# serhii-rieznik/metal-renderer

Hardware: AMD Instinct MI355X
Metric: Mpaths/s at 1920×1080, 4 bounces; achieved HBM GB/s vs peak; 1/2/4/8-GPU scaling (higher is better)
Workload: dtype f32

## Files before the change

### include/mrt.h

```cpp
#ifndef MRT_H_
#define MRT_H_

#include <stddef.h>
#include <stdint.h>

#ifdef __cplusplus
extern "C" {
#endif

#define MRT_ABI_VERSION 9

typedef enum mrt_status {
  MRT_OK = 0,
  MRT_ERR_INVALID = -1,
  MRT_ERR_IO = -2,
  MRT_ERR_HIP = -3,
  MRT_ERR_NOMEM = -4,
  MRT_ERR_STATE = -5,
  MRT_ERR_COMM = -6
} mrt_status;

#define MRT_FLAG_PRECISE 1u
#define MRT_FLAG_PROFILE 2u
#define MRT_FLAG_STATIC_NOISE 4u
// ... 188 lines not shown
int mrt_renderer_destroy(mrt_renderer* r);

const char* mrt_last_error(void);
int mrt_abi_version(void);
int mrt_noise_table(uint64_t seed, int64_t frame, float* out16384);
int mrt_shard_mask(uint32_t width, uint32_t height, uint32_t shard_rank, uint32_t shard_count, uint8_t* mask,
                   uint64_t* owned);
#define MRT_DISPLAY_TONEMAP 1u
#define MRT_DISPLAY_SRGB 2u
#define MRT_DISPLAY_DENOISED 4u
#define MRT_DISPLAY_RESOLVED 8u
#define MRT_DISPLAY_COMPARE(mode) ((uint32_t)(mode) << 8)
int mrt_display(const float* image, const float* reference, float* out, uint32_t width, uint32_t height,
                uint32_t flags, float compare_scale, void* stream);

int mrt_image_load_exr(const char* path, float* rgba, size_t capacity_floats, uint32_t* width, uint32_t* height);
int mrt_renderer_load_reference(mrt_renderer* r, const char* path);
int mrt_renderer_display(mrt_renderer* r, uint32_t flags, float compare_scale, float* rgba, size_t count);
#define MRT_DISPLAY_SLOTS 3u
int mrt_renderer_display_enqueue(mrt_renderer* r, uint32_t flags, float compare_scale, uint32_t slot);
int mrt_renderer_display_map(mrt_renderer* r, uint32_t slot, const float** rgba, size_t* count);

int mrt_tiles_packed_floats(uint32_t width, uint32_t height, uint32_t shard_rank, uint32_t shard_count,
                            uint64_t* floats);
int mrt_tiles_pack(const float* image, uint32_t width, uint32_t height, uint32_t shard_rank,
                   uint32_t shard_count, float* packed, void* stream);
int mrt_tiles_unpack(const float* packed, uint32_t width, uint32_t height, uint32_t shard_rank,
                     uint32_t shard_count, float* image, void* stream);
#define MRT_COMM_ID_BYTES 128
#define MRT_EXCHANGE_GATHER 1u
#define MRT_EXCHANGE_REDUCE 2u
#define MRT_EXCHANGE_OVERLAP 0x100u
typedef struct mrt_comm mrt_comm;
int mrt_comm_unique_id(void* id, size_t bytes);
int mrt_comm_create(const void* id, uint32_t nranks, uint32_t rank, int device, mrt_comm** out);
int mrt_comm_destroy(mrt_comm* comm);
int mrt_renderer_exchange(mrt_renderer* r, mrt_comm* comm, uint32_t mode);
int mrt_renderer_exchange_flush(mrt_renderer* r);
int mrt_comm_set_timeout(mrt_comm* comm, uint32_t timeout_ms);
int mrt_comm_check(mrt_comm* comm);
int mrt_debug_comm_fail(mrt_comm* comm, uint32_t mode);
int mrt_renderer_tiles_read(mrt_renderer* r, float* host_packed, size_t floats);
int mrt_renderer_tiles_write(mrt_renderer* r, uint32_t shard_rank, const float* host_packed, size_t floats);

int mrt_synchronize(void* stream);
int mrt_event_record(void* stream, void** event);
int mrt_event_synchronize(void* event);
int mrt_event_destroy(void* event);
int mrt_debug_stamps(uint64_t* out8, int reset);
int mrt_debug_wave_times(uint64_t* out, size_t n);
int mrt_debug_lanes(uint64_t* out, size_t n, int reset);
int mrt_debug_sweep_list(const mrt_scene* scene, float* records, uint32_t capacity, uint32_t* count,
                         uint32_t* enabled);
int mrt_debug_sweep_cap(const mrt_scene* scene, uint32_t* cap);
int mrt_debug_bvh_nodes(const mrt_scene* scene, float* nodes, uint32_t capacity, uint32_t* count);
int mrt_debug_exchange_unpack(mrt_renderer* r, uint32_t nranks, const float* gathered, size_t floats);
int mrt_debug_box_margin(const mrt_scene* scene, const void* rays, uint32_t stride, uint32_t count,
                         const void* intersections, float* out);
int mrt_debug_magic_div(uint32_t d, const uint32_t* n, uint32_t count, uint32_t* q);
int mrt_debug_denoise_path(uint32_t path);
int mrt_debug_denoise_step(const float* image, const float* guide_n, const float* guide_p, float* out, float* scratch,
                           uint32_t width, uint32_t height, const mrt_denoise_params* params, uint32_t step_log2,
                           uint32_t path, void* stream);
int mrt_device_count(void);

#ifdef __cplusplus
}
#endif
#endif
```

### metal-renderer_amd/csrc/kernels.hip

```cpp
#include <hip/hip_runtime.h>
#include <math.h>

#include <algorithm>
#include <cstdlib>
#include <vector>

#include "diag_env.h"
#include "kernels.h"

#ifndef MRT_PRECISE
#error "compile with -DMRT_PRECISE=0 or 1"
#endif
#ifndef MRT_TU
#define MRT_TU 0
#endif
#ifndef MRT_LANESTATS
#define MRT_LANESTATS 0
#endif
#define MRT_EMIT_STREAM (MRT_TU == 0 || (MRT_TU == 2 && !MRT_LANESTATS) || (MRT_TU == 1 && MRT_LANESTATS))
#define MRT_EMIT_MAIN (MRT_TU != 2)
#if MRT_PRECISE
#define MRT_NS precise
#else
#define MRT_NS fast
// ... 290 lines not shown
  return (int32_t)v;
}

template <int MODE>
__device__ __forceinline__ LdsCtx stage_lds(const DeviceScene& sc, uint32_t scratch_u32, uint32_t* spill = nullptr) {
  LdsCtx cx;
  const uint32_t nf4 = node_float4s(sc.width);
  const uint32_t n_nodes = (MODE == kAllLds) ? scene_nodes(sc) : (MODE == kTopLds ? sc.lds_nodes : 0u);
  const uint32_t TR = (MODE == kAllLds) ? scene_tri_records(sc) : 0u;
  const uint32_t T = (MODE == kAllLds) ? sc.num_triangles : 0u;
  const uint32_t M = (MODE == kAllLds) ? sc.num_materials : 0u;
  const uint32_t NL = (MODE == kAllLds) ? sc.num_lights + 1 : 0u;
  const uint32_t SW = (MODE == kAllLds) ? sc.sweep_leaves : 0u;
  cx.n_lds_nodes = n_nodes;
  const uint32_t node_f4 = node_stride_f4(MODE, nf4);
  const bool copies = node_f4 != nf4;
  cx.tri_base = node_f4 * n_nodes;
  cx.prim_base = cx.tri_base + 3 * TR;
  cx.mat_base = cx.prim_base + 6 * T;
  cx.light_base = cx.mat_base + 2 * M;
  cx.sweep_base = cx.light_base + 7 * NL;
  const uint32_t f4 = cx.sweep_base + 2 * SW;
  cx.scratch_base = 4 * f4;
  cx.stack_base = cx.scratch_base + ((scratch_u32 + 3) & ~3u);
  cx.spill_lane = sc.max_stack;
  cx.spill = spill ? spill + (size_t)blockIdx.x * kBlock * cx.spill_lane : nullptr;
  if (MODE != kGlobal) {
    const float4* src[6] = {reinterpret_cast<const float4*>(sc.nodes), reinterpret_cast<const float4*>(sc.tris),
                            reinterpret_cast<const float4*>(sc.prims), reinterpret_cast<const float4*>(sc.materials),
                            reinterpret_cast<const float4*>(sc.lights), reinterpret_cast<const float4*>(sc.sweep)};
    const uint32_t base[6] = {0u, cx.tri_base, cx.prim_base, cx.mat_base, cx.light_base, cx.sweep_base};
    const uint32_t len[6] = {nf4 * n_nodes, 3 * TR, 6 * T, 2 * M, 7 * NL, 2 * SW};
    for (int r = copies ? 1 : 0; r < 6; ++r)
      for (uint32_t i = threadIdx.x; i < len[r]; i += kBlock) g_lds[base[r] + i] = src[r][i];
    if (copies) {
      for (uint32_t i = threadIdx.x; i < node_f4 * n_nodes; i += kBlock) {
        const uint32_t node = i / node_f4, rem = i % node_f4;
        const uint32_t quad = rem / kQuadCopyF4, row = rem % kQuadCopyF4;
        const uint32_t axis = row >> 1;
        const uint32_t flip = axis < 2 ? (quad >> axis) & 1u : 0u;
        const uint32_t src_row = row < 6 ? 2 * axis + ((row & 1u) ^ flip) : 6u;
        g_lds[i] = src[0][8 * node + src_row];
      }
    }
    __syncthreads();
  }
  return cx;
}

#ifndef MRT_LANESTATS
#define MRT_LANESTATS 0
#endif
#if MRT_LANESTATS
constexpr int kLaneStats = 46;
__shared__ unsigned long long s_lanes[kBlock / 64][kLaneStats];
__device__ unsigned long long g_lanes[kLaneStats];
__device__ __forceinline__ void ls_add(int k, uint32_t v) {
  const uint64_t m = __ballot(1);
  if ((threadIdx.x & 63u) == (uint32_t)(__ffsll((unsigned long long)m) - 1)) s_lanes[threadIdx.x >> 6][k] += v;
}
__device__ __forceinline__ uint32_t ls_lanes() { return (uint32_t)__popcll(__ballot(1)); }
#define LS_ADD(k, v) ls_add((k), (v))
#define LS_INIT() do { if ((threadIdx.x & 63u) < (uint32_t)kLaneStats) s_lanes[threadIdx.x >> 6][threadIdx.x & 63u] = 0; } while (0)
#define LS_FLUSH() do { const uint32_t l_ = threadIdx.x & 63u; \
    if (l_ < (uint32_t)kLaneStats && s_lanes[threadIdx.x >> 6][l_]) atomicAdd(&g_lanes[l_], s_lanes[threadIdx.x >> 6][l_]); } while (0)
__device__ __forceinline__ uint64_t ls_clock() {
  uint64_t t;
  asm volatile("s_memtime %0\n\ts_waitcnt lgkmcnt(0)" : "=s"(t)::"memory");
  return t;
}
#define LS_T0() const uint64_t ls_t0_ = ls_clock()
#define LS_T1(k) do { LS_ADD((k), (uint32_t)(ls_clock() - ls_t0_)); LS_ADD((k) + 1, 1); } while (0)
#define LS_WAIT_VM(k) do { LS_T0(); asm volatile("s_waitcnt vmcnt(0)" ::: "memory"); LS_T1(k); } while (0)
#else
#define LS_ADD(k, v) do {} while (0)
#define LS_INIT() do {} while (0)
#define LS_FLUSH() do {} while (0)
#define LS_T0() do {} while (0)
#define LS_T1(k) do {} while (0)
#define LS_WAIT_VM(k) do {} while (0)
#endif

constexpr int32_t kDone = 0x7FFFFFFF;
#ifndef MRT_PATH_SLACK
#define MRT_PATH_SLACK 16
#endif
#ifndef MRT_LEAF_SLACK
#define MRT_LEAF_SLACK 12
#endif

template <int STACK>
__device__ __forceinline__ int32_t stack_pop(const LdsCtx& cx, int& sp) {
  if (STACK < 0 && !__any(sp > (STACK < 0 ? -STACK : STACK))) {
    const int32_t n = sp > 0 ? (int32_t)lds_u32()[cx.stack_base + threadIdx.x + (sp - 1) * kBlock] : kDone;
    sp = max(sp - 1, 0);
    return n;
  }
  const int32_t n = sp > 0 ? stack_get<STACK>(cx, sp - 1) : kDone;
  sp = max(sp - 1, 0);
  return n;
}

[[maybe_unused]] constexpr float kCullScale = 1.0f + 0x1p-11f;
template <int STACK, int MODE, bool ANY>
__device__ __forceinline__ int32_t interior_step(const DeviceScene& sc, const LdsCtx& cx, int32_t node, V3 o,
                                                 const RayBox& rb, float tmin, float tmax, int& sp) {
  {
// ... 101 lines not shown
  h.prim = 0xFFFFFFFFu;
  h.found = false;
  for (uint32_t j = 0; j < cnt; j += 2) {
    const uint32_t j1 = min(j + 1, cnt - 1);
#if MRT_LANESTATS
    const uint64_t t0_ = ls_clock();
    const uint32_t e0_ = list[j], e1_ = list[j1];
    asm volatile("s_waitcnt lgkmcnt(0)" ::"s"(e0_), "s"(e1_) : "memory");
    LS_ADD(38, (uint32_t)(ls_clock() - t0_));
#endif
    tri_pair<MODE>(sc, cx, o, d, 0.0f, list[j], list[j1], j1 != j, h, false, 0u, nullptr);
  }
}

template <int STACK, int MODE, bool ANY>
__device__ __forceinline__ bool traverse(const DeviceScene& sc, const LdsCtx& cx, V3 o, V3 d, float tmin, Hit& h,
                                         uint32_t target, int32_t root) {
  const RayBox rb = make_raybox(o, d);
  int32_t node = root, leaf = 0;
  int sp = 0;
  constexpr int kLs = ANY ? 6 : 0;
  (void)kLs;
  LS_ADD(kLs + 0, ls_lanes());
  LS_ADD(kLs + 1, 1);
  if (node < 0) { leaf = node; node = kDone; }
  while (node != kDone || leaf != 0) {
    while (node != kDone && node >= 0) {
      LS_ADD(kLs + 2, 1);
      LS_ADD(kLs + 3, ls_lanes());
      node = interior_step<STACK, MODE, ANY>(sc, cx, node, o, rb, tmin, h.t, sp);
      if (node < 0 && leaf == 0) {
        leaf = node;
        node = stack_pop<STACK>(cx, sp);
      }
      if (__ballot(leaf == 0) == 0ull) break;
    }
    while (leaf < 0) {
      LS_ADD(kLs + 4, 1);
      LS_ADD(kLs + 5, ls_lanes());
      const uint32_t lr = ~(uint32_t)leaf;
      const uint32_t first = lr >> kLeafCountBits, cnt = (lr & (kMaxLeafSize - 1)) + 1;
      if (leaf_tests<MODE>(sc, cx, o, d, tmin, first, cnt, h, ANY, target, nullptr)) return true;
      leaf = 0;
      if (node < 0) {
        leaf = node;
        node = stack_pop<STACK>(cx, sp);
      }
    }
  }
  return false;
}


__device__ __forceinline__ bool sweep_box(float4 lo, float4 hi, V3 o, const RayBox& rb, float tmin, float& tnear) {
#if MRT_PRECISE
  const float ox = o.x, oy = o.y, oz = o.z, oix = 0.0f, oiy = 0.0f, oiz = 0.0f;
#else
  const float ox = 0.0f, oy = 0.0f, oz = 0.0f, oix = rb.oinv.x, oiy = rb.oinv.y, oiz = rb.oinv.z;
  (void)o;
#endif
  const float x0 = slab(lo.x, ox, rb.inv.x, oix), x1 = slab(hi.x, ox, rb.inv.x, oix);
  const float y0 = slab(lo.y, oy, rb.inv.y, oiy), y1 = slab(hi.y, oy, rb.inv.y, oiy);
  const float z0 = slab(lo.z, oz, rb.inv.z, oiz), z1 = slab(hi.z, oz, rb.inv.z, oiz);
  tnear = fmaxf(fmaxf(fminf(x0, x1), fminf(y0, y1)), fmaxf(fminf(z0, z1), tmin));
  const float tfar = fminf(fminf(fmaxf(x0, x1), fmaxf(y0, y1)), fmaxf(z0, z1));
  return tnear <= tfar;
}

typedef float SweepRec __attribute__((ext_vector_type(8)));
typedef const __attribute__((address_space(4))) SweepRec* SweepList;

template <int MODE>
__device__ __forceinline__ void sweep_leaf(const DeviceScene& sc, const LdsCtx& cx, V3 o, V3 d, float tmin,
                                           uint32_t ref, Hit& h) {
  LS_ADD(4, 1);
  LS_ADD(5, ls_lanes());
  const uint32_t lr = ~ref;
  leaf_tests<MODE>(sc, cx, o, d, tmin, lr >> kLeafCountBits, (lr & (kMaxLeafSize - 1)) + 1, h, false, 0u, nullptr);
}

template <int MODE, bool CAP = false>
__device__ __forceinline__ uint32_t sweep_nearest(const DeviceScene& sc, const LdsCtx& cx, V3 o, V3 d, float tmin,
                                                  Hit& h, uint32_t cap = 0xFFFFFFFFu, uint32_t resume = 0u) {
  const RayBox rb = make_raybox(o, d);
  LS_ADD(0, ls_lanes());
  LS_ADD(1, 1);
  constexpr uint32_t kNone = 0xFFFFFFFFu;
  uint32_t k1 = kNone, k2 = kNone, rest = 0u;
  const uint32_t n = sc.sweep_leaves;
  const SweepList list = (SweepList)(uintptr_t)sc.sweep;
  for (uint32_t i = 0; i < n; ++i) {
    LS_T0();
    const SweepRec rec = list[i];
#if MRT_LANESTATS
    asm volatile("" ::"s"(rec[0]), "s"(rec[7]));
    LS_T1(42);
#endif
    float te;
    const bool hit = sweep_box(make_float4(rec[0], rec[1], rec[2], rec[3]), make_float4(rec[4], rec[5], rec[6], rec[7]),
                               o, rb, tmin, te);
    const uint32_t key = hit ? ((fbits(te) & ~31u) | (i & 31u)) : kNone;
    const uint32_t mid = max(k1, key);
    k1 = min(k1, key);
    k2 = min(k2, mid);
    rest |= (hit ? 1u : 0u) << (i & 31u);
  }
  rest &= ~((1u << (k1 & 31u)) | (1u << (k2 & 31u)));
  auto pop = [&](uint32_t& ref) {
    const uint32_t id = (uint32_t)__ffs((int)rest) - 1u;
    rest &= rest - 1u;
    const float4 blo = g_lds[cx.sweep_base + 2u * id], bhi = g_lds[cx.sweep_base + 2u * id + 1u];
    float te;
    ref = fbits(blo.w);
    return sweep_box(blo, bhi, o, rb, tmin, te) && te <= h.t * kCullScale;
  };
  if (!CAP) {
    if (k1 != kNone) sweep_leaf<MODE>(sc, cx, o, d, tmin, fbits(g_lds[cx.sweep_base + 2u * (k1 & 31u)].w), h);
    if (k2 != kNone && bitsf(k2 & ~31u) <= h.t * kCullScale)
      sweep_leaf<MODE>(sc, cx, o, d, tmin, fbits(g_lds[cx.sweep_base + 2u * (k2 & 31u)].w), h);
  } else {
    if (resume) rest = resume;
#pragma unroll
    for (int round = 0; round < 2; ++round) {
      const uint32_t k = round == 0 ? k1 : k2;
      bool test = k != kNone && (round == 0 || bitsf(k & ~31u) <= h.t * kCullScale);
      uint32_t ref = 0u;
      if (resume) {
        test = false;
        if (rest) test = pop(ref);
      } else if (test) {
        ref = fbits(g_lds[cx.sweep_base + 2u * (k & 31u)].w);
      }
      if (test) sweep_leaf<MODE>(sc, cx, o, d, tmin, ref, h);
    }
  }
  for (uint32_t c = 0; rest && (!CAP || c < cap); ++c) {
    LS_ADD(30, 1);
    LS_ADD(31, ls_lanes());
    uint32_t ref;
    if (pop(ref)) sweep_leaf<MODE>(sc, cx, o, d, tmin, ref, h);
  }
  return CAP ? rest : 0u;
}

template <int STACK, int MODE>
__device__ __forceinline__ Hit trace_nearest(const DeviceScene& sc, const LdsCtx& cx, V3 o, V3 d, float tmin,
                                             float tmax) {
  Hit h;
  h.t = tmax;
  h.u = h.v = 0.0f;
  h.prim = 0xFFFFFFFFu;
  h.found = false;
  if (MODE == kAllLds && sc.sweep_leaves) {
    sweep_nearest<MODE>(sc, cx, o, d, tmin, h);
    return h;
  }
  traverse<STACK, MODE, false>(sc, cx, o, d, tmin, h, 0u, sc.root);
  return h;
}

__device__ __forceinline__ int32_t shadow_root(const DeviceScene& sc, V3 o, bool graze) {
  const int32_t main_root = __builtin_amdgcn_readfirstlane(sc.root);
  if (sc.occ_planes == 0) return main_root;
  const int32_t occ_root = __builtin_amdgcn_readfirstlane(sc.occ_root);
  bool inside = !graze;
  for (uint32_t k = 0; k < sc.occ_planes; ++k) {
    const float* p = sc.occ_plane[k];
    inside &= fmaf(p[0], o.x, fmaf(p[1], o.y, fmaf(p[2], o.z, -p[3]))) <= -sc.occ_margin;
  }
  return inside ? occ_root : main_root;
}
__device__ __forceinline__ int32_t shadow_root_select(const DeviceScene& sc, V3 o, bool graze) {
  if (sc.occ_planes == 0 || graze) return sc.root;
  bool inside = true;
  for (uint32_t k = 0; k < sc.occ_planes; ++k) {
    const float* p = sc.occ_plane[k];
    inside &= fmaf(p[0], o.x, fmaf(p[1], o.y, fmaf(p[2], o.z, -p[3]))) <= -sc.occ_margin;
  }
  return inside ? sc.occ_root : sc.root;
}

template <int MODE>
__device__ __forceinline__ bool lights_occlude(const DeviceScene& sc, const LdsCtx& cx, V3 o, V3 d, uint32_t target,
                                               uint32_t tl, float tT) {
  bool occ = false;
  for (uint32_t j = 0; j + 1 < sc.num_lights; ++j) {
// ... 1872 lines not shown
```

### metal-renderer_amd/csrc/renderer.cpp

```cpp
#include <hip/hip_runtime.h>
#include <rccl/rccl.h>

#include <algorithm>
#include <atomic>
#include <chrono>
#include <cmath>
#include <cstdio>
#include <cstdlib>
#include <cstring>
#include <memory>
#include <mutex>
#include <string>
#include <thread>
#include <vector>

#include "../../include/mrt.h"
#include "bvh.h"
#include "bvh_gpu.h"
#include "denoise.h"
#include "temporal.h"
#include "image.h"
#include "kernels.h"
#include "noise.h"
#include "noise_schedule.h"
#include "occluders.h"
#include "primary.h"
#include "scene.h"
#include "diag_env.h"

namespace {

thread_local std::string g_last_error;

int fail(int code, const std::string& msg) {
  g_last_error = msg;
  return code;
}

#define HIP_TRY(expr)                                                                             \
  do {                                                                                            \
    hipError_t e_ = (expr);                                                                       \
    if (e_ != hipSuccess)                                                                         \
      return fail(MRT_ERR_HIP, std::string(#expr) + ": " + hipGetErrorString(e_));                \
  } while (0)

inline float bitsf(uint32_t u) { float f; std::memcpy(&f, &u, 4); return f; }
inline uint32_t fbits(float f) { uint32_t u; std::memcpy(&u, &f, 4); return u; }

struct DevBuf {
  void* p = nullptr;
  size_t bytes = 0;
  ~DevBuf() { if (p) (void)hipFree(p); }
  hipError_t alloc(size_t n) {
    if (p) { (void)hipFree(p); p = nullptr; }
    bytes = n;
    return n ? hipMalloc(&p, n) : hipSuccess;
  }
  template <class T> T* as() const { return reinterpret_cast<T*>(p); }
};

hipError_t alloc_isect_spill(DevBuf& b, uint32_t max_stack) {
  if (max_stack <= (uint32_t)mrt::kMaxStack) return b.alloc(0);
  return b.alloc((size_t)max_stack * mrt::kIntersectSpillGrid * 256 * 4);
}

#define NCCL_TRY(expr)                                                                            \
  do {                                                                                            \
    ncclResult_t e_ = (expr);                                                                     \
    if (e_ != ncclSuccess)                                                                        \
      return fail(MRT_ERR_HIP, std::string(#expr) + ": " + ncclGetErrorString(e_));               \
  } while (0)

hipError_t upload(DevBuf& b, const void* src, size_t n) {
  hipError_t e = b.alloc(std::max<size_t>(n, 16));
  if (e != hipSuccess) return e;
  return n ? hipMemcpy(b.p, src, n, hipMemcpyHostToDevice) : hipSuccess;
}

}

struct mrt_accel {
  mrt_accel_desc desc{};
  DevBuf nodes, tris;
  DevBuf isect_spill;
  mrt::DeviceScene dev{};
  mrt_accel_info info{};
};

struct mrt_scene {
  int device = 0;
  DevBuf isect_spill;
  mrt::HostScene host;
  mrt::BvhResult bvh;
  std::vector<float> occ_nodes, occ_tris;
  std::vector<uint32_t> occ_keep;
  int32_t occ_root = 0;
  uint32_t occ_node_base = 0, occ_max_stack = 0;
  DevBuf nodes, tris, prims, materials, lights;
  std::vector<float> sweep_list;
  bool sweep_on = false;
  uint32_t sweep_cap = mrt::kSweepCap;
  DevBuf sweep;
  mrt::DeviceScene dev{};
  mrt_scene_info info{};
};

struct DrawRecord {
  DevBuf counters;
  hipEvent_t start = nullptr, stop = nullptr;
  hipEvent_t cleared = nullptr;
  hipEvent_t copied = nullptr;
  void* host = nullptr;
  void* host_dev = nullptr;
  size_t host_bytes = 0;
  std::vector<hipEvent_t> kernel_events;
  uint32_t frames = 0;
  uint32_t launches = 0;
  size_t span_off = 0;
  size_t counter_bytes = 0;
  size_t events = 0;
  bool pending = false;
  bool clean = false;
};
constexpr int kDrawRing = 3;

struct FrameSlot {
  hipStream_t stream = nullptr;
  bool own_stream = false;
  DevBuf queue[2][mrt::kQueuePlanes];
  DevBuf segments;
  DevBuf radiance;
  DevBuf spill;
  hipEvent_t acc_done = nullptr;
  hipEvent_t kernel_done = nullptr;
  bool acc_recorded = false;
};

struct CameraGen {
  DevBuf dev;
  void* host = nullptr;
  size_t host_bytes = 0;
  hipEvent_t ready = nullptr;
  hipEvent_t retired = nullptr;
  bool busy = false;
  bool async = false;
  uint32_t waited_streams = 0;
  bool moved = false;
  bool has_lists = false;
  uint32_t primary_bx = 0;
  ~CameraGen() {
    if (ready) (void)hipEventDestroy(ready);
    if (retired) (void)hipEventDestroy(retired);
// ... 781 lines not shown
      occ_root = mrt::kEmptyChild;
    } else {
      if (ob.num_nodes) up_nodes.insert(up_nodes.end(), ob.nodes.begin(), ob.nodes.begin() + 32 * (size_t)ob.num_nodes);
      up_tris.insert(up_tris.end(), ob.tris.begin(), ob.tris.end());
      s->occ_nodes.assign(ob.nodes.begin(), ob.nodes.begin() + 32 * (size_t)ob.num_nodes);
      s->occ_tris = ob.tris;
      s->occ_keep = occ.keep;
      s->occ_root = occ_root;
      s->occ_node_base = node_base;
      s->occ_max_stack = ob.max_stack;
    }
  }
  mrt::ConvexSet conv;
  bool conv_on = occ_on && occ_lights && occ_root != mrt::kEmptyChild;
  if (const char* v = mrt::diag_env("MRT_CONVEX")) conv_on = conv_on && std::atoi(v) != 0;
  if (conv_on)
    conv_on = mrt::find_convex_occluders(h.vertices.data()->v, sizeof(mrt::RefVertex), (uint32_t)h.vertices.size(),
                                         h.indices.data(), T, occ.keep, occ, conv);
  if (conv_on)
    for (uint32_t t = 0; t < T; ++t) {
      const uint32_t code = conv.prim_face[t];
      prims[(size_t)t * 24 + 11] = bitsf(code);
      if (code)
        for (int c = 0; c < 3; ++c) prims[(size_t)t * 24 + 15 + 4 * c] = conv.face_normal[(code - 1) / 8][3 * ((code - 1) % 8) + c];
    }
  mrt_scene_info& in = s->info;
  if (conv_on) {
    in.convex_solids = conv.count;
    in.convex_delta = conv.delta;
    for (uint32_t c = 0; c < conv.count; ++c) {
      for (int i = 0; i < 16; ++i) in.convex_obb[c][i] = conv.obb[c][i];
      for (int k = 0; k < 8; ++k) in.convex_face_tris[c][k] = conv.face_tris[c][k];
    }
  }
  if (occ_on) {
    in.occluder_planes = (uint32_t)occ.planes.size();
    in.occluder_culled = occ.culled;
    in.occluder_nodes = ob.num_nodes;
    in.occluder_margin = occ.margin;
    in.occluder_max_stack = ob.max_stack;
    in.occluder_cos_min = occ.cos_min;
    for (size_t k = 0; k < occ.planes.size() && k < 8; ++k)
      for (int c = 0; c < 4; ++c) in.occluder_plane[k][c] = occ.planes[k][c];
  }
  if (s->bvh.root >= 0 && s->bvh.num_leaves <= mrt::kSweepLeaves) {
    for (uint32_t k = 0; k < s->bvh.num_nodes; ++k) {
      const float* nd = &s->bvh.nodes[32 * (size_t)k];
      for (int c = 0; c < 4; ++c)
        if ((int32_t)fbits(nd[24 + c]) < 0)
          s->sweep_list.insert(s->sweep_list.end(), {nd[c], nd[8 + c], nd[16 + c], nd[24 + c],
                                                     nd[4 + c], nd[12 + c], nd[20 + c], 0.0f});
    }
  }
  const uint32_t sweep_leaves = (uint32_t)(s->sweep_list.size() / 8);
  const uint32_t up_occ_nodes = occ_on ? (uint32_t)(up_nodes.size() / 32) - s->bvh.num_nodes : 0u;
  if (sweep_leaves >= 1 && sweep_leaves <= mrt::kSweepLeaves && s->bvh.width == 4) {
    mrt::DeviceScene probe{};
    probe.num_nodes = s->bvh.num_nodes;
    probe.num_triangles = T;
    probe.num_materials = (uint32_t)h.materials.size();
    probe.num_lights = h.light_count;
    probe.lds_nodes = s->bvh.lds_nodes;
    probe.width = s->bvh.width;
    probe.occ_nodes = up_occ_nodes;
    probe.occ_tris = occ_on ? (uint32_t)occ.keep.size() : 0u;
    probe.sweep_leaves = sweep_leaves;
    s->sweep_on = !mrt::fast::path_preferred(probe);
  }
  if (const char* v = mrt::diag_env("MRT_SWEEP")) s->sweep_on = s->sweep_on && std::atoi(v) != 0;
  if (const char* v = mrt::diag_env("MRT_SWEEP_CAP"))
    s->sweep_cap = (uint32_t)std::min<unsigned long>(std::strtoul(v, nullptr, 0), mrt::kSweepLeaves);
  in.vertices = (uint32_t)h.vertices.size();
  in.triangles = T;
  in.materials = (uint32_t)h.materials.size();
  in.light_triangles = h.light_count;
  in.bvh_nodes = s->bvh.num_nodes;
  in.bvh_leaves = s->bvh.num_leaves;
  in.bvh_depth = s->bvh.max_depth;
  in.bvh_lds_nodes = s->bvh.lds_nodes;
  in.bvh_width = s->bvh.width;
  in.bvh_max_stack = s->bvh.max_stack;
  in.bvh_sah_cost = s->bvh.sah_cost;
  in.build_ms = build_ms;
  if (desc->device < 0) {
    *out = s.release();
    return MRT_OK;
  }
  if ((uint64_t)up_nodes.size() * 4 >= (1ull << 32) || (uint64_t)up_tris.size() * 4 >= (1ull << 32) ||
      (uint64_t)s->bvh.nodes.size() * 4 >= (1ull << 32) || (uint64_t)T * 48 >= (1ull << 32))
    return fail(MRT_ERR_INVALID, "scene too large: BVH nodes or leaf triangles exceed 4 GiB");
  HIP_TRY(hipSetDevice(desc->device));
  if (builder == MRT_BVH_HOST_SAH) {
    HIP_TRY(upload(s->nodes, up_nodes.data(), up_nodes.size() * 4));
    HIP_TRY(upload(s->tris, up_tris.data(), up_tris.size() * 4));
  }
  HIP_TRY(upload(s->prims, prims.data(), prims.size() * 4));
  HIP_TRY(upload(s->materials, mats.data(), mats.size() * 4));
  HIP_TRY(upload(s->lights, lights.data(), lights.size() * 4));
  mrt::DeviceScene& d = s->dev;
  d.nodes = s->nodes.as<float>();
  d.tris = s->tris.as<float>();
  d.prims = s->prims.as<float>();
  d.materials = s->materials.as<float>();
  d.lights = s->lights.as<float>();
  d.root = s->bvh.root;
  d.num_nodes = s->bvh.num_nodes;
  d.num_triangles = T;
  d.num_materials = (uint32_t)h.materials.size();
  d.num_lights = h.light_count;
  d.lds_nodes = s->bvh.lds_nodes;
  d.width = s->bvh.width;
  d.max_stack = s->bvh.max_stack;
  d.origin_test = T >= mrt::kOriginTestTriangles ? 1u : 0u;
  if (const char* v = mrt::diag_env("MRT_ORIGIN_TEST")) d.origin_test = std::atoi(v) != 0;
  d.region_grabs = T >= mrt::kRegionGrabTriangles ? 1u : 0u;
  if (const char* v = mrt::diag_env("MRT_REGIONS")) d.region_grabs = std::atoi(v) != 0;
  d.light_shortcut = h.light_count <= mrt::kLightShortcutMax ? 1u : 0u;
  if (const char* v = mrt::diag_env("MRT_LAST_LIGHT")) d.light_shortcut = d.light_shortcut && std::atoi(v) != 0;
  d.occ_root = occ_root;
  d.occ_planes = 0;
  d.occ_lights = 0;
  if (occ_on) {
    d.occ_lights = occ_lights ? 1u : 0u;
    d.occ_nodes = up_occ_nodes;
    d.occ_tris = (uint32_t)occ.keep.size();
    d.occ_planes = (uint32_t)occ.planes.size();
    d.occ_margin = occ.margin;
    d.occ_cos_min = occ.cos_min;
    d.occ_cos_min2 = occ.cos_min * occ.cos_min;
    for (uint32_t k = 0; k < d.occ_planes; ++k)
      for (int c = 0; c < 4; ++c) d.occ_plane[k][c] = occ.planes[k][c];
    d.max_stack = std::max(d.max_stack, ob.max_stack);
  }
  d.conv_count = in.convex_solids;
  std::memcpy(d.conv_obb, in.convex_obb, sizeof(d.conv_obb));
  std::memcpy(d.conv_face_tris, in.convex_face_tris, sizeof(d.conv_face_tris));
  d.sweep = nullptr;
  d.sweep_leaves = 0;
  d.sweep_cap = s->sweep_cap;
  if (s->sweep_on) {
    HIP_TRY(upload(s->sweep, s->sweep_list.data(), s->sweep_list.size() * 4));
    d.sweep = s->sweep.as<float>();
    d.sweep_leaves = sweep_leaves;
  }
  HIP_TRY(alloc_isect_spill(s->isect_spill, d.max_stack));
  in.device_bytes = s->nodes.bytes + s->tris.bytes + s->prims.bytes + s->materials.bytes + s->lights.bytes +
                    s->sweep.bytes;
  *out = s.release();
  return MRT_OK;
}

int mrt_scene_info_get(const mrt_scene* scene, mrt_scene_info* info) {
  if (!scene || !info) return fail(MRT_ERR_INVALID, "null argument");
  *info = scene->info;
  return MRT_OK;
}

int mrt_debug_sweep_list(const mrt_scene* scene, float* records, uint32_t capacity, uint32_t* count,
                         uint32_t* enabled) {
  if (!scene || !count || !enabled) return fail(MRT_ERR_INVALID, "mrt_debug_sweep_list: null argument");
  const uint32_t n = (uint32_t)(scene->sweep_list.size() / 8);
  if (records) std::memcpy(records, scene->sweep_list.data(), (size_t)std::min(n, capacity) * 32);
  *count = n;
  *enabled = scene->sweep_on ? 1u : 0u;
  return MRT_OK;
}

int mrt_debug_sweep_cap(const mrt_scene* scene, uint32_t* cap) {
  if (!scene || !cap) return fail(MRT_ERR_INVALID, "mrt_debug_sweep_cap: null argument");
  *cap = scene->sweep_cap;
  return MRT_OK;
}

int mrt_debug_bvh_nodes(const mrt_scene* scene, float* nodes, uint32_t capacity, uint32_t* count) {
  if (!scene || !count) return fail(MRT_ERR_INVALID, "mrt_debug_bvh_nodes: null argument");
  const uint32_t n = scene->bvh.num_nodes;
  if (nodes) std::memcpy(nodes, scene->bvh.nodes.data(), (size_t)std::min(n, capacity) * 128);
  *count = n;
  return MRT_OK;
}

int mrt_scene_export(const mrt_scene* scene, void* vertices, void* indices, void* materials, void* references,
                     void* lights) {
  if (!scene) return fail(MRT_ERR_INVALID, "null scene");
  const mrt::HostScene& h = scene->host;
  if (vertices) std::memcpy(vertices, h.vertices.data(), h.vertices.size() * sizeof(mrt::RefVertex));
  if (indices) std::memcpy(indices, h.indices.data(), h.indices.size() * 4);
  if (materials) std::memcpy(materials, h.materials.data(), h.materials.size() * sizeof(mrt::RefMaterial));
  if (references) std::memcpy(references, h.references.data(), h.references.size() * sizeof(mrt::RefTriangleReference));
  if (lights) std::memcpy(lights, h.lights.data(), h.lights.size() * sizeof(mrt::RefLightTriangle));
  return MRT_OK;
}

extern "C++" {
namespace {
template <class NodeFn, class TriFn>
int check_tree(const mrt::HostScene& h, int32_t root, uint32_t node_lo, uint32_t num_nodes, uint32_t tri_lo,
               uint32_t tri_count, uint32_t max_stack, const std::vector<uint8_t>& want, NodeFn node, TriFn tri,
               const char* what) {
  const uint32_t T = (uint32_t)h.references.size();
  std::vector<uint8_t> seen(T, 0);
  auto fbits = [](float f) { uint32_t u; std::memcpy(&u, &f, 4); return u; };
  auto bad = [&](const char* m) { return fail(MRT_ERR_STATE, std::string(what) + ": " + m); };
  struct Item { int32_t ref; float lo[3], hi[3]; uint32_t depth, pend; };
  std::vector<Item> stack;
  stack.push_back(Item{root, {-1e30f, -1e30f, -1e30f}, {1e30f, 1e30f, 1e30f}, 0, 0});
  uint32_t nodes_seen = 0;
  while (!stack.empty()) {
    Item it = stack.back();
    stack.pop_back();
    if (it.depth >= (uint32_t)mrt::kMaxTraversalStack) return bad("BVH too deep");
    if (it.ref >= 0) {
      if ((uint32_t)it.ref < node_lo || (uint32_t)it.ref - node_lo >= num_nodes) return bad("BVH node index out of range");
      ++nodes_seen;
      Item ch[4];
      uint32_t nc = 0;
      {
// ... 1611 lines not shown
```

### metal-renderer_amd/mrt.py

```python
from __future__ import annotations

import ctypes
import os
import subprocess

HERE = os.path.dirname(os.path.abspath(__file__))
LIB_PATH = os.environ.get("MRT_LIB") or os.path.join(HERE, "lib", "libmrt.so")
INCLUDE_H = os.path.join(os.path.dirname(HERE), "include", "mrt.h")
SCENES_DIR = os.path.join(HERE, "scenes")

FLAG_PRECISE = 1
FLAG_PROFILE = 2
FLAG_STATIC_NOISE = 4
FLAG_NO_ACCUMULATE = 8
FLAG_DEBUG_MATERIAL = 16
COMM_ID_BYTES = 128
EXCHANGE_GATHER, EXCHANGE_REDUCE, EXCHANGE_OVERLAP = 1, 2, 0x100
DEFAULT_SEED = 0x6D6574616C2D7274

RAY_BYTES, SHADOW_RAY_BYTES, ISECT_BYTES = 80, 48, 16


class MrtError(RuntimeError):
    pass
# ... 120 lines not shown

class DenoiseParams(ctypes.Structure):
    _fields_ = [
        ("iterations", ctypes.c_uint32), ("sigma_color", ctypes.c_float), ("sigma_plane", ctypes.c_float),
        ("normal_log2_power", ctypes.c_uint32),
    ]

    @classmethod
    def default(cls, frames: int) -> "DenoiseParams":
        p = cls()
        _check(lib().mrt_denoise_params_default(frames, ctypes.byref(p)), "mrt_denoise_params_default")
        return p

    def check(self) -> None:
        _check(lib().mrt_denoise_params_check(ctypes.byref(self)), "mrt_denoise_params_check")

    def as_dict(self) -> dict:
        return {k: getattr(self, k) for k, _ in self._fields_}


class ReprojectParams(ctypes.Structure):
    _fields_ = [
        ("plane_tolerance", ctypes.c_float), ("normal_cos_min", ctypes.c_float), ("max_history", ctypes.c_float),
    ]

    @classmethod
    def default(cls) -> "ReprojectParams":
        p = cls()
        _check(lib().mrt_reproject_params_default(ctypes.byref(p)), "mrt_reproject_params_default")
        return p

    def check(self) -> None:
        _check(lib().mrt_reproject_params_check(ctypes.byref(self)), "mrt_reproject_params_check")

    def as_dict(self) -> dict:
        return {k: getattr(self, k) for k, _ in self._fields_}


EXPORTED = [
    "mrt_scene_create", "mrt_scene_info_get", "mrt_scene_export", "mrt_scene_destroy", "mrt_scene_check_bvh",
    "mrt_raygen", "mrt_intersect", "mrt_shade", "mrt_resolve_shadow", "mrt_accumulate",
    "mrt_renderer_create", "mrt_renderer_resize", "mrt_renderer_reset", "mrt_renderer_prepare",
    "mrt_renderer_draw", "mrt_renderer_draw_n", "mrt_renderer_sync", "mrt_renderer_image", "mrt_renderer_stream",
    "mrt_renderer_read_image", "mrt_renderer_save_image", "mrt_renderer_stats", "mrt_renderer_destroy",
    "mrt_last_error", "mrt_abi_version", "mrt_noise_table", "mrt_device_count", "mrt_synchronize",
    "mrt_event_record", "mrt_event_synchronize", "mrt_event_destroy",
    "mrt_debug_stamps", "mrt_debug_wave_times", "mrt_shard_mask",
    "mrt_tiles_packed_floats", "mrt_tiles_pack", "mrt_tiles_unpack", "mrt_display", "mrt_renderer_set_max_frames",
    "mrt_accel_create", "mrt_accel_rebuild", "mrt_accel_intersect", "mrt_accel_info_get", "mrt_accel_destroy",
    "mrt_comm_unique_id", "mrt_comm_create", "mrt_comm_destroy", "mrt_renderer_exchange",
    "mrt_renderer_exchange_flush", "mrt_renderer_tiles_read", "mrt_renderer_tiles_write",
    "mrt_image_load_exr", "mrt_renderer_load_reference", "mrt_renderer_display",
    "mrt_renderer_display_enqueue", "mrt_renderer_display_map",
    "mrt_debug_lanes", "mrt_debug_sweep_list", "mrt_debug_sweep_cap", "mrt_debug_bvh_nodes", "mrt_debug_exchange_unpack", "mrt_debug_box_margin",
    "mrt_debug_magic_div", "mrt_comm_set_timeout", "mrt_comm_check", "mrt_debug_comm_fail",
    "mrt_camera_default", "mrt_camera_look_at", "mrt_camera_check", "mrt_raygen_camera",
    "mrt_renderer_set_camera", "mrt_renderer_get_camera",
    "mrt_guides", "mrt_denoise_params_default", "mrt_denoise_params_check", "mrt_denoise",
    "mrt_renderer_denoise", "mrt_renderer_read_denoised", "mrt_renderer_save_denoised", "mrt_debug_denoise_path",
    "mrt_debug_denoise_step",
    "mrt_reproject_params_default", "mrt_reproject_params_check", "mrt_temporal_resolve", "mrt_reproject",
    "mrt_renderer_move_camera", "mrt_renderer_resolve", "mrt_renderer_read_resolved", "mrt_renderer_save_resolved",
    "mrt_renderer_denoise_resolved",
]

_lib = None


def build(jobs: int = 4) -> None:
    subprocess.run(["make", "-s", f"-j{jobs}", "-C", HERE], check=True)


def lib() -> ctypes.CDLL:
    global _lib
    if _lib is not None:
        return _lib
    if not os.path.exists(LIB_PATH):
        raise MrtError(f"native library missing: {LIB_PATH} (run __graft_entry__.build())")
    L = ctypes.CDLL(LIB_PATH)
    vp, u32, u64, i64, c_int = ctypes.c_void_p, ctypes.c_uint32, ctypes.c_uint64, ctypes.c_int64, ctypes.c_int
    sig = {
        "mrt_scene_create": [ctypes.POINTER(SceneDesc), ctypes.POINTER(vp)],
        "mrt_scene_info_get": [vp, ctypes.POINTER(SceneInfo)],
        "mrt_scene_export": [vp, vp, vp, vp, vp, vp],
        "mrt_scene_destroy": [vp],
        "mrt_scene_check_bvh": [vp],
        "mrt_raygen": [vp, u32, u32, vp, vp, u32, vp],
        "mrt_intersect": [vp, vp, u32, u32, vp, u32, vp],
        "mrt_shade": [vp, u32, u32, u32, u32, vp, vp, vp, vp, u32, vp],
        "mrt_resolve_shadow": [vp, u32, vp, vp, vp, u32, vp],
        "mrt_accumulate": [vp, u32, u32, u32, vp, vp, u32, vp],
        "mrt_renderer_create": [ctypes.POINTER(RendererDesc), ctypes.POINTER(vp)],
        "mrt_renderer_resize": [vp, u32, u32],
        "mrt_renderer_reset": [vp],
        "mrt_renderer_prepare": [vp, u32],
        "mrt_renderer_draw": [vp],
        "mrt_renderer_draw_n": [vp, u32],
        "mrt_renderer_sync": [vp],
        "mrt_renderer_image": [vp, ctypes.POINTER(vp)],
        "mrt_renderer_stream": [vp, ctypes.POINTER(vp)],
        "mrt_renderer_read_image": [vp, vp, ctypes.c_size_t],
        "mrt_renderer_save_image": [vp, ctypes.c_char_p],
        "mrt_renderer_stats": [vp, ctypes.POINTER(Stats)],
        "mrt_renderer_destroy": [vp],
        "mrt_last_error": [],
        "mrt_abi_version": [],
        "mrt_noise_table": [u64, i64, vp],
        "mrt_device_count": [],
        "mrt_synchronize": [vp],
        "mrt_event_record": [vp, ctypes.POINTER(vp)],
        "mrt_event_synchronize": [vp],
        "mrt_event_destroy": [vp],
        "mrt_debug_stamps": [vp, c_int],
        "mrt_debug_wave_times": [vp, ctypes.c_size_t],
        "mrt_debug_lanes": [vp, ctypes.c_size_t, c_int],
        "mrt_debug_sweep_list": [vp, vp, u32, vp, vp],
        "mrt_debug_sweep_cap": [vp, vp],
        "mrt_debug_bvh_nodes": [vp, vp, u32, vp],
        "mrt_debug_exchange_unpack": [vp, u32, vp, ctypes.c_size_t],
        "mrt_debug_box_margin": [vp, vp, u32, u32, vp, vp],
        "mrt_debug_magic_div": [u32, vp, u32, vp],
        "mrt_comm_set_timeout": [vp, u32],
        "mrt_comm_check": [vp],
        "mrt_debug_comm_fail": [vp, u32],
        "mrt_shard_mask": [u32, u32, u32, u32, vp, vp],
        "mrt_tiles_packed_floats": [u32, u32, u32, u32, ctypes.POINTER(u64)],
        "mrt_display": [vp, vp, vp, u32, u32, u32, ctypes.c_float, vp],
        "mrt_renderer_set_max_frames": [vp, u32],
        "mrt_tiles_pack": [vp, u32, u32, u32, u32, vp, vp],
        "mrt_tiles_unpack": [vp, u32, u32, u32, u32, vp, vp],
        "mrt_accel_create": [ctypes.POINTER(AccelDesc), ctypes.POINTER(vp)],
        "mrt_accel_rebuild": [vp],
        "mrt_accel_intersect": [vp, vp, u32, u32, vp, u32, vp],
        "mrt_accel_info_get": [vp, ctypes.POINTER(AccelInfo)],
        "mrt_accel_destroy": [vp],
        "mrt_comm_unique_id": [vp, ctypes.c_size_t],
        "mrt_comm_create": [vp, u32, u32, c_int, ctypes.POINTER(vp)],
        "mrt_comm_destroy": [vp],
        "mrt_renderer_exchange": [vp, vp, u32],
        "mrt_renderer_exchange_flush": [vp],
        "mrt_renderer_tiles_read": [vp, vp, ctypes.c_size_t],
        "mrt_renderer_tiles_write": [vp, u32, vp, ctypes.c_size_t],
        "mrt_image_load_exr": [ctypes.c_char_p, vp, ctypes.c_size_t, ctypes.POINTER(u32), ctypes.POINTER(u32)],
        "mrt_renderer_load_reference": [vp, ctypes.c_char_p],
        "mrt_renderer_display": [vp, u32, ctypes.c_float, vp, ctypes.c_size_t],
        "mrt_renderer_display_enqueue": [vp, u32, ctypes.c_float, u32],
        "mrt_renderer_display_map": [vp, u32, ctypes.POINTER(ctypes.c_void_p), ctypes.POINTER(ctypes.c_size_t)],
        "mrt_camera_default": [ctypes.POINTER(Camera)],
        "mrt_camera_look_at": [ctypes.c_float * 3, ctypes.c_float * 3, ctypes.c_float * 3, ctypes.c_float,
                               ctypes.POINTER(Camera)],
        "mrt_camera_check": [ctypes.POINTER(Camera)],
        "mrt_raygen_camera": [vp, ctypes.POINTER(Camera), u32, u32, vp, vp, u32, vp],
        "mrt_renderer_set_camera": [vp, ctypes.POINTER(Camera)],
        "mrt_renderer_get_camera": [vp, ctypes.POINTER(Camera)],
        "mrt_guides": [vp, ctypes.POINTER(Camera), u32, u32, vp, vp, u32, vp],
        "mrt_denoise_params_default": [u64, ctypes.POINTER(DenoiseParams)],
        "mrt_denoise_params_check": [ctypes.POINTER(DenoiseParams)],
        "mrt_denoise": [vp, vp, vp, vp, vp, u32, u32, ctypes.POINTER(DenoiseParams), vp],
        "mrt_renderer_denoise": [vp, ctypes.POINTER(DenoiseParams)],
        "mrt_renderer_read_denoised": [vp, vp, ctypes.c_size_t],
        "mrt_renderer_save_denoised": [vp, ctypes.c_char_p],
        "mrt_debug_denoise_path": [u32],
        "mrt_debug_denoise_step": [vp, vp, vp, vp, vp, u32, u32, ctypes.POINTER(DenoiseParams), u32, u32, vp],
        "mrt_reproject_params_default": [ctypes.POINTER(ReprojectParams)],
        "mrt_reproject_params_check": [ctypes.POINTER(ReprojectParams)],
        "mrt_temporal_resolve": [vp, u64, vp, vp, u32, u32, vp],
        "mrt_reproject": [vp, vp, vp, ctypes.POINTER(Camera), vp, vp, vp, u32, u32, ctypes.POINTER(ReprojectParams), vp],
        "mrt_renderer_move_camera": [vp, ctypes.POINTER(Camera), ctypes.POINTER(ReprojectParams)],
        "mrt_renderer_resolve": [vp],
# ... 453 lines not shown
    import numpy as np
    H, W = image.shape[:2]
    tx_n, ty_n = (W + 63) // 64, (H + 63) // 64
    tiles = list(range(rank, tx_n * ty_n, count))
    out = np.zeros((len(tiles), 64, 64, 4), np.float32)
    for k, t in enumerate(tiles):
        ty, tx = divmod(t, tx_n)
        blk = image[ty * 64:(ty + 1) * 64, tx * 64:(tx + 1) * 64]
        out[k, :blk.shape[0], :blk.shape[1]] = blk
    return out


def tiles_unpack_host(packed, image, rank: int, count: int) -> None:
    H, W = image.shape[:2]
    tx_n, ty_n = (W + 63) // 64, (H + 63) // 64
    for k, t in enumerate(range(rank, tx_n * ty_n, count)):
        ty, tx = divmod(t, tx_n)
        h, w = min(64, H - ty * 64), min(64, W - tx * 64)
        image[ty * 64:ty * 64 + h, tx * 64:tx * 64 + w] = packed[k, :h, :w]


def debug_magic_div(d: int, n):
    import numpy as np
    n = np.ascontiguousarray(n, np.uint32)
    q = np.zeros(len(n), np.uint32)
    _check(lib().mrt_debug_magic_div(d, ctypes.c_void_p(n.ctypes.data), len(n), ctypes.c_void_p(q.ctypes.data)),
           "mrt_debug_magic_div")
    return q


def debug_stamps(reset: bool = True):
    import numpy as np
    out = np.zeros(8, np.uint64)
    _check(lib().mrt_debug_stamps(ctypes.c_void_p(out.ctypes.data), int(reset)), "mrt_debug_stamps")
    return out


def debug_lanes(reset: bool = True):
    import numpy as np
    out = np.zeros(64, np.uint64)
    _check(lib().mrt_debug_lanes(ctypes.c_void_p(out.ctypes.data), out.size, int(reset)), "mrt_debug_lanes")
    return out


def debug_sweep_list(scene: "Scene"):
    import numpy as np
    out = np.zeros((32, 8), np.uint32)
    count, enabled = ctypes.c_uint32(), ctypes.c_uint32()
    _check(lib().mrt_debug_sweep_list(scene.handle, ctypes.c_void_p(out.ctypes.data), len(out), ctypes.byref(count),
                                      ctypes.byref(enabled)), "mrt_debug_sweep_list")
    return bool(enabled.value), out[:min(count.value, len(out))].copy()


def debug_sweep_cap(scene: "Scene") -> int:
    cap = ctypes.c_uint32()
    _check(lib().mrt_debug_sweep_cap(scene.handle, ctypes.byref(cap)), "mrt_debug_sweep_cap")
    return cap.value


def debug_bvh_nodes(scene: "Scene"):
    import numpy as np
    out = np.zeros((scene.info["bvh_nodes"], 32), np.uint32)
    count = ctypes.c_uint32()
    _check(lib().mrt_debug_bvh_nodes(scene.handle, ctypes.c_void_p(out.ctypes.data), len(out), ctypes.byref(count)),
           "mrt_debug_bvh_nodes")
    return out[:count.value]


def debug_wave_times():
    import numpy as np
    out = np.zeros((4, 8192, 16), np.uint64)
    _check(lib().mrt_debug_wave_times(ctypes.c_void_p(out.ctypes.data), out.size), "mrt_debug_wave_times")
    return out


class Event:

    def __init__(self):
        self._e = ctypes.c_void_p()

    def record(self, stream=None) -> None:
        _check(lib().mrt_event_record(stream, ctypes.byref(self._e)), "mrt_event_record")

    def synchronize(self) -> None:
        _check(lib().mrt_event_synchronize(self._e), "mrt_event_synchronize")

    def close(self) -> None:
        if self._e.value:
            _check(lib().mrt_event_destroy(self._e), "mrt_event_destroy")
            self._e = ctypes.c_void_p()


def load_exr(path: str):
    import numpy as np
    w, h = ctypes.c_uint32(), ctypes.c_uint32()
    _check(lib().mrt_image_load_exr(path.encode(), None, 0, ctypes.byref(w), ctypes.byref(h)), "mrt_image_load_exr")
    img = np.zeros((h.value, w.value, 4), np.float32)
    _check(lib().mrt_image_load_exr(path.encode(), ctypes.c_void_p(img.ctypes.data), img.size, ctypes.byref(w),
                                    ctypes.byref(h)), "mrt_image_load_exr")
    return img


def comm_unique_id() -> bytes:
    buf = ctypes.create_string_buffer(COMM_ID_BYTES)
    _check(lib().mrt_comm_unique_id(buf, COMM_ID_BYTES), "mrt_comm_unique_id")
    return buf.raw
# ... 42 lines not shown
```

Baseline: 14070.

## Rebuild sweep list as triangle-pair records and generalize sweep key selection

Converts the flat sweep leaf list into records that each hold at most two triangles, greedily merging single-triangle leaves whose union box has less surface area than the two separate boxes. The kernel then runs a fixed pair test per record instead of a variable-length leaf loop. It also makes the number of nearest keys tracked (two or three) a compile-time option and adds early termination of the remaining-hit mask once a key fails the distance cull. The aim is to cut divergent leaf loops and box tests, at the cost of possibly more records when large leaves are split and looser merged boxes.

```diff
diff --git a/include/mrt.h b/include/mrt.h
--- a/include/mrt.h
+++ b/include/mrt.h
@@ -264,6 +264,8 @@
 int mrt_debug_lanes(uint64_t* out, size_t n, int reset);
 int mrt_debug_sweep_list(const mrt_scene* scene, float* records, uint32_t capacity, uint32_t* count,
                          uint32_t* enabled);
+int mrt_debug_sweep_pairs(const mrt_scene* scene, float* records, uint32_t* prims, uint32_t capacity,
+                          uint32_t* count);
 int mrt_debug_sweep_cap(const mrt_scene* scene, uint32_t* cap);
 int mrt_debug_bvh_nodes(const mrt_scene* scene, float* nodes, uint32_t capacity, uint32_t* count);
 int mrt_debug_exchange_unpack(mrt_renderer* r, uint32_t nranks, const float* gathered, size_t floats);
diff --git a/metal-renderer_amd/csrc/kernels.hip b/metal-renderer_amd/csrc/kernels.hip
--- a/metal-renderer_amd/csrc/kernels.hip
+++ b/metal-renderer_amd/csrc/kernels.hip
@@ -366,7 +366,7 @@
 #define MRT_LANESTATS 0
 #endif
 #if MRT_LANESTATS
-constexpr int kLaneStats = 46;
+constexpr int kLaneStats = 48;
 __shared__ unsigned long long s_lanes[kBlock / 64][kLaneStats];
 __device__ unsigned long long g_lanes[kLaneStats];
 __device__ __forceinline__ void ls_add(int k, uint32_t v) {
@@ -574,6 +574,14 @@
 }
 
 
+#ifndef MRT_SWEEP_KEYS
+#define MRT_SWEEP_KEYS 2
+#endif
+#ifndef MRT_SWEEP_EARLY
+#define MRT_SWEEP_EARLY 1
+#endif
+constexpr int kSweepKeys = MRT_SWEEP_KEYS;
+static_assert(kSweepKeys == 2 || kSweepKeys == 3, "MRT_SWEEP_KEYS");
 __device__ __forceinline__ bool sweep_box(float4 lo, float4 hi, V3 o, const RayBox& rb, float tmin, float& tnear) {
 #if MRT_PRECISE
   const float ox = o.x, oy = o.y, oz = o.z, oix = 0.0f, oiy = 0.0f, oiz = 0.0f;
@@ -597,8 +605,8 @@
                                            uint32_t ref, Hit& h) {
   LS_ADD(4, 1);
   LS_ADD(5, ls_lanes());
-  const uint32_t lr = ~ref;
-  leaf_tests<MODE>(sc, cx, o, d, tmin, lr >> kLeafCountBits, (lr & (kMaxLeafSize - 1)) + 1, h, false, 0u, nullptr);
+  const uint32_t ka = ref & 0xFFFFu, kb = ref >> 16;
+  tri_pair<MODE>(sc, cx, o, d, tmin, ka, kb, kb != ka, h, false, 0u, nullptr);
 }
 
 template <int MODE, bool CAP = false>
@@ -608,7 +616,8 @@
   LS_ADD(0, ls_lanes());
   LS_ADD(1, 1);
   constexpr uint32_t kNone = 0xFFFFFFFFu;
-  uint32_t k1 = kNone, k2 = kNone, rest = 0u;
+  uint32_t key_of[3] = {kNone, kNone, kNone};
+  uint32_t rest = 0u;
   const uint32_t n = sc.sweep_leaves;
   const SweepList list = (SweepList)(uintptr_t)sc.sweep;
   for (uint32_t i = 0; i < n; ++i) {
@@ -621,13 +630,22 @@
     float te;
     const bool hit = sweep_box(make_float4(rec[0], rec[1], rec[2], rec[3]), make_float4(rec[4], rec[5], rec[6], rec[7]),
                                o, rb, tmin, te);
-    const uint32_t key = hit ? ((fbits(te) & ~31u) | (i & 31u)) : kNone;
-    const uint32_t mid = max(k1, key);
-    k1 = min(k1, key);
-    k2 = min(k2, mid);
+    const uint32_t key = hit ? ((fbits(te) & 0x7FFFFFE0u) | (i & 31u)) : kNone;
+    const uint32_t mid = max(key_of[0], key);
+    key_of[0] = min(key_of[0], key);
+    if (kSweepKeys == 3) {
+      key_of[2] = min(key_of[2], max(key_of[1], mid));
+      key_of[1] = min(key_of[1], mid);
+    } else {
+      key_of[1] = min(key_of[1], mid);
+    }
     rest |= (hit ? 1u : 0u) << (i & 31u);
   }
-  rest &= ~((1u << (k1 & 31u)) | (1u << (k2 & 31u)));
+  {
+    uint32_t keyed = (1u << (key_of[0] & 31u)) | (1u << (key_of[1] & 31u));
+    if (kSweepKeys == 3) keyed |= 1u << (key_of[2] & 31u);
+    rest &= ~keyed;
+  }
   auto pop = [&](uint32_t& ref) {
     const uint32_t id = (uint32_t)__ffs((int)rest) - 1u;
     rest &= rest - 1u;
@@ -636,24 +654,26 @@
     ref = fbits(blo.w);
     return sweep_box(blo, bhi, o, rb, tmin, te) && te <= h.t * kCullScale;
   };
-  if (!CAP) {
-    if (k1 != kNone) sweep_leaf<MODE>(sc, cx, o, d, tmin, fbits(g_lds[cx.sweep_base + 2u * (k1 & 31u)].w), h);
-    if (k2 != kNone && bitsf(k2 & ~31u) <= h.t * kCullScale)
-      sweep_leaf<MODE>(sc, cx, o, d, tmin, fbits(g_lds[cx.sweep_base + 2u * (k2 & 31u)].w), h);
-  } else {
-    if (resume) rest = resume;
+  if (CAP && resume) rest = resume;
 #pragma unroll
-    for (int round = 0; round < 2; ++round) {
-      const uint32_t k = round == 0 ? k1 : k2;
-      bool test = k != kNone && (round == 0 || bitsf(k & ~31u) <= h.t * kCullScale);
-      uint32_t ref = 0u;
-      if (resume) {
-        test = false;
-        if (rest) test = pop(ref);
-      } else if (test) {
-        ref = fbits(g_lds[cx.sweep_base + 2u * (k & 31u)].w);
+  for (int round = 0; round < kSweepKeys; ++round) {
+    const uint32_t k = key_of[round];
+    bool test = round == 0 ? k != kNone : bitsf(k & ~31u) <= h.t * kCullScale;
+    uint32_t ref = 0u;
+    if (CAP && resume) {
+      test = false;
+      if (rest) test = pop(ref);
+    } else if (test) {
+      ref = fbits(g_lds[cx.sweep_base + 2u * (k & 31u)].w);
+    } else if (MRT_SWEEP_EARLY) {
+      rest = 0u;
+    }
+    if (test) {
+      if (round == 2) {
+        LS_ADD(46, 1);
+        LS_ADD(47, ls_lanes());
       }
-      if (test) sweep_leaf<MODE>(sc, cx, o, d, tmin, ref, h);
+      sweep_leaf<MODE>(sc, cx, o, d, tmin, ref, h);
     }
   }
   for (uint32_t c = 0; rest && (!CAP || c < cap); ++c) {
diff --git a/metal-renderer_amd/csrc/renderer.cpp b/metal-renderer_amd/csrc/renderer.cpp
--- a/metal-renderer_amd/csrc/renderer.cpp
+++ b/metal-renderer_amd/csrc/renderer.cpp
@@ -26,6 +26,7 @@
 #include "occluders.h"
 #include "primary.h"
 #include "scene.h"
+#include "sweep_pairs.h"
 #include "diag_env.h"
 
 namespace {
@@ -97,7 +98,7 @@
   int32_t occ_root = 0;
   uint32_t occ_node_base = 0, occ_max_stack = 0;
   DevBuf nodes, tris, prims, materials, lights;
-  std::vector<float> sweep_list;
+  std::vector<float> sweep_list, sweep_pairs;
   bool sweep_on = false;
   uint32_t sweep_cap = mrt::kSweepCap;
   DevBuf sweep;
@@ -985,7 +986,10 @@
                                                      nd[4 + c], nd[12 + c], nd[20 + c], 0.0f});
     }
   }
-  const uint32_t sweep_leaves = (uint32_t)(s->sweep_list.size() / 8);
+  bool pair_singles = true;
+  if (const char* v = mrt::diag_env("MRT_SWEEP_PAIRS")) pair_singles = std::atoi(v) != 0;
+  mrt::sweep_pair_records(s->sweep_list, pair_singles, s->sweep_pairs);
+  const uint32_t sweep_leaves = (uint32_t)(s->sweep_pairs.size() / 8);
   const uint32_t up_occ_nodes = occ_on ? (uint32_t)(up_nodes.size() / 32) - s->bvh.num_nodes : 0u;
   if (sweep_leaves >= 1 && sweep_leaves <= mrt::kSweepLeaves && s->bvh.width == 4) {
     mrt::DeviceScene probe{};
@@ -1072,7 +1076,7 @@
   d.sweep_leaves = 0;
   d.sweep_cap = s->sweep_cap;
   if (s->sweep_on) {
-    HIP_TRY(upload(s->sweep, s->sweep_list.data(), s->sweep_list.size() * 4));
+    HIP_TRY(upload(s->sweep, s->sweep_pairs.data(), s->sweep_pairs.size() * 4));
     d.sweep = s->sweep.as<float>();
     d.sweep_leaves = sweep_leaves;
   }
@@ -1096,6 +1100,21 @@
   if (records) std::memcpy(records, scene->sweep_list.data(), (size_t)std::min(n, capacity) * 32);
   *count = n;
   *enabled = scene->sweep_on ? 1u : 0u;
+  return MRT_OK;
+}
+
+int mrt_debug_sweep_pairs(const mrt_scene* scene, float* records, uint32_t* prims, uint32_t capacity,
+                          uint32_t* count) {
+  if (!scene || !count) return fail(MRT_ERR_INVALID, "mrt_debug_sweep_pairs: null argument");
+  const uint32_t n = (uint32_t)(scene->sweep_pairs.size() / 8), m = std::min(n, capacity);
+  if (records) std::memcpy(records, scene->sweep_pairs.data(), (size_t)m * 32);
+  if (prims)
+    for (uint32_t i = 0; i < m; ++i) {
+      const uint32_t w = fbits(scene->sweep_pairs[8 * (size_t)i + 3]);
+      prims[2 * i] = fbits(scene->bvh.tris[12 * (size_t)(w & 0xFFFFu) + 3]);
+      prims[2 * i + 1] = fbits(scene->bvh.tris[12 * (size_t)(w >> 16) + 3]);
+    }
+  *count = n;
   return MRT_OK;
 }
 
diff --git a/metal-renderer_amd/csrc/sweep_pairs.h b/metal-renderer_amd/csrc/sweep_pairs.h
--- /dev/null
+++ b/metal-renderer_amd/csrc/sweep_pairs.h
@@ -0,0 +1,70 @@
+#pragma once
+#include <algorithm>
+#include <cstdint>
+#include <cstring>
+#include <vector>
+
+#include "mrt_layout.h"
+
+namespace mrt {
+
+inline void sweep_pair_records(const std::vector<float>& leaves, bool pair_singles, std::vector<float>& out) {
+  out.clear();
+  const int n = (int)(leaves.size() / 8);
+  auto bits = [&](int i) { uint32_t u; std::memcpy(&u, &leaves[8 * (size_t)i + 3], 4); return ~u; };
+  auto first = [&](int i) { return bits(i) >> kLeafCountBits; };
+  auto count = [&](int i) { return (bits(i) & (uint32_t)(kMaxLeafSize - 1)) + 1u; };
+  auto area = [](const float* lo, const float* hi) {
+    const double x = (double)hi[0] - lo[0], y = (double)hi[1] - lo[1], z = (double)hi[2] - lo[2];
+    return x * y + y * z + z * x;
+  };
+  auto unite = [&](int i, int j, float* lo, float* hi) {
+    for (int a = 0; a < 3; ++a) {
+      lo[a] = std::min(leaves[8 * (size_t)i + a], leaves[8 * (size_t)j + a]);
+      hi[a] = std::max(leaves[8 * (size_t)i + 4 + a], leaves[8 * (size_t)j + 4 + a]);
+    }
+  };
+  for (int i = 0; i < n; ++i)
+    if (first(i) + count(i) > 0x10000u) return;
+  std::vector<int> mate(n, -1);
+  while (pair_singles) {
+    int bi = -1, bj = -1;
+    double best = 0.0;
+    for (int i = 0; i < n; ++i) {
+      if (count(i) != 1 || mate[i] >= 0) continue;
+      for (int j = i + 1; j < n; ++j) {
+        if (count(j) != 1 || mate[j] >= 0) continue;
+        float lo[3], hi[3];
+        unite(i, j, lo, hi);
+        const double a = area(lo, hi);
+        if (!(a < area(&leaves[8 * (size_t)i], &leaves[8 * (size_t)i + 4]) +
+                      area(&leaves[8 * (size_t)j], &leaves[8 * (size_t)j + 4])))
+          continue;
+        if (bi < 0 || a < best) { bi = i; bj = j; best = a; }
+      }
+    }
+    if (bi < 0) break;
+    mate[bi] = bj;
+    mate[bj] = bi;
+  }
+  auto emit = [&](const float* lo, const float* hi, uint32_t ka, uint32_t kb) {
+    const uint32_t w = ka | (kb << 16);
+    float wf;
+    std::memcpy(&wf, &w, 4);
+    out.insert(out.end(), {lo[0], lo[1], lo[2], wf, hi[0], hi[1], hi[2], 0.0f});
+  };
+  for (int i = 0; i < n; ++i) {
+    const float *lo = &leaves[8 * (size_t)i], *hi = lo + 4;
+    const uint32_t f = first(i), cnt = count(i);
+    if (mate[i] >= 0) {
+      if (mate[i] < i) continue;
+      float ulo[3], uhi[3];
+      unite(i, mate[i], ulo, uhi);
+      emit(ulo, uhi, f, first(mate[i]));
+      continue;
+    }
+    for (uint32_t k = 0; k < cnt; k += 2) emit(lo, hi, f + k, f + std::min(k + 1, cnt - 1));
+  }
+}
+
+}
diff --git a/metal-renderer_amd/mrt.py b/metal-renderer_amd/mrt.py
--- a/metal-renderer_amd/mrt.py
+++ b/metal-renderer_amd/mrt.py
@@ -196,7 +196,7 @@
     "mrt_renderer_exchange_flush", "mrt_renderer_tiles_read", "mrt_renderer_tiles_write",
     "mrt_image_load_exr", "mrt_renderer_load_reference", "mrt_renderer_display",
     "mrt_renderer_display_enqueue", "mrt_renderer_display_map",
-    "mrt_debug_lanes", "mrt_debug_sweep_list", "mrt_debug_sweep_cap", "mrt_debug_bvh_nodes", "mrt_debug_exchange_unpack", "mrt_debug_box_margin",
+    "mrt_debug_lanes", "mrt_debug_sweep_list", "mrt_debug_sweep_pairs", "mrt_debug_sweep_cap", "mrt_debug_bvh_nodes", "mrt_debug_exchange_unpack", "mrt_debug_box_margin",
     "mrt_debug_magic_div", "mrt_comm_set_timeout", "mrt_comm_check", "mrt_debug_comm_fail",
     "mrt_camera_default", "mrt_camera_look_at", "mrt_camera_check", "mrt_raygen_camera",
     "mrt_renderer_set_camera", "mrt_renderer_get_camera",
@@ -259,6 +259,7 @@
         "mrt_debug_wave_times": [vp, ctypes.c_size_t],
         "mrt_debug_lanes": [vp, ctypes.c_size_t, c_int],
         "mrt_debug_sweep_list": [vp, vp, u32, vp, vp],
+        "mrt_debug_sweep_pairs": [vp, vp, vp, u32, vp],
         "mrt_debug_sweep_cap": [vp, vp],
         "mrt_debug_bvh_nodes": [vp, vp, u32, vp],
         "mrt_debug_exchange_unpack": [vp, u32, vp, ctypes.c_size_t],
@@ -818,6 +819,17 @@
     return bool(enabled.value), out[:min(count.value, len(out))].copy()
 
 
+def debug_sweep_pairs(scene: "Scene"):
+    import numpy as np
+    out, prims = np.zeros((32, 8), np.uint32), np.zeros((32, 2), np.uint32)
+    count = ctypes.c_uint32()
+    _check(lib().mrt_debug_sweep_pairs(scene.handle, ctypes.c_void_p(out.ctypes.data),
+                                       ctypes.c_void_p(prims.ctypes.data), len(out), ctypes.byref(count)),
+           "mrt_debug_sweep_pairs")
+    n = min(count.value, len(out))
+    return out[:n].copy(), prims[:n].copy()
+
+
 def debug_sweep_cap(scene: "Scene") -> int:
     cap = ctypes.c_uint32()
     _check(lib().mrt_debug_sweep_cap(scene.handle, ctypes.byref(cap)), "mrt_debug_sweep_cap")
```

Result: faster. 15100 (median of 6 runs) (+7.3%).
